# SonyCSLParis/interactive-spectrogram-inpainting

Hardware: AMD Instinct MI355X
Metric: spectrograms/sec VQ-VAE fwd+quantize @B64 (higher is better)
Workload: dtype f32 (products split into two f16 pieces, three terms); 1 GPU; VQVAE.forward (encode + quantize x2 + decode), eval, default ctor (128 hidden, 2 res blocks, D=64, K=512, factors 4/2); batch_per_gpu=64, input=[2,128,512] fp32 randn, weights=random init, codebooks calibrated on encoder outputs, parallelism=replicas x1 (no data-path collective)

## Files before the change

interactive-spectrogram-inpainting_amd/csrc/convT_pair_f16.hip:

```cpp
#include "isi_common.h"
#include "isi_internal.h"
#include "knobs.h"
#include "prof.h"
#include "split_f16.h"

namespace isi {

namespace {

typedef float f32x16 __attribute__((ext_vector_type(16)));
typedef int i32x4 __attribute__((ext_vector_type(4)));
typedef short s16x8 __attribute__((ext_vector_type(8)));
typedef unsigned u32x2v __attribute__((ext_vector_type(2)));
using f16s::f16x8;

constexpr int TW = 64, HWD = TW + 2;
constexpr int ROWB = 64;
constexpr int NPAIR = 8;
constexpr unsigned OOB = 0x7FFFFFF0u, OOB_ST = 0xFFFFFFF0u;

struct ConvTPairK {
  const float *in, *w16, *bias;
  float *out;
  unsigned in_bytes, w_bytes, out_bytes;
  int Cin, Cout, Kpad, H, W, B, relu;
  int tiles_x, tiles_y, ntn;
  const float *w2;
  int n2;
  float *out2;
};

__device__ __forceinline__ void dma16(const unsigned lds_addr, const unsigned voff, const i32x4 rsrc, const unsigned soff) {
  asm volatile("s_mov_b32 m0, %0\n\ts_nop 0\n\tbuffer_load_dwordx4 %1, %2, %3 offen lds"
               :: "s"(lds_addr), "v"(voff), "s"(rsrc), "s"(soff) : "memory");
}
__device__ __forceinline__ i32x4 make_rsrc(const void *ptr, const unsigned bytes) {
  const unsigned long long b = (unsigned long long)ptr;
  return i32x4{(int)(unsigned)b, (int)((unsigned)(b >> 32) & 0xffffu), (int)bytes, 0x00020000};
}
#ifdef ISI_MEASURE
__device__ long long g_convT_pair_stamps[128];
#define ISI_STAMP(i_) do { if (blockIdx.x == 8 && (wave & 3) == 0 && lane == 0 && item_i == (int)blockIdx.x + (int)gridDim.x) \
    g_convT_pair_stamps[(wave >> 2) * 64 + (i_)] = __builtin_readcyclecounter(); } while (0)
#else
#define ISI_STAMP(i_) do { } while (0)
#endif
#define ISI_MH(a_, b_, c_) __builtin_amdgcn_mfma_f32_32x32x16_f16(__builtin_bit_cast(f16x8, a_), __builtin_bit_cast(f16x8, b_), c_, 0, 0, 0)

template <int TH, bool OUTP, bool YP = false>
__global__ __launch_bounds__(TH * 64) void convT_pair_kernel(const ConvTPairK p) {
  constexpr int NW = TH;
  constexpr int HPIX = (TH + 1) * HWD;
  constexpr int A_ROWS = (HPIX + 15) / 16 * 16;
  constexpr int NA = A_ROWS / 16, NWD = NPAIR * 64 / 16;
  constexpr int A_BYTES = A_ROWS * ROWB, W_BYTES = NPAIR * 64 * ROWB, STAGE = A_BYTES + W_BYTES + 1024;
  constexpr int NS = 2;
  constexpr int NDMA = NA + NWD;
  constexpr int PER = (NDMA + NW - 1) / NW;
  extern __shared__ __attribute__((aligned(16))) char smem[];

  const int tid = threadIdx.x, lane = tid & 63;
  const int wave = __builtin_amdgcn_readfirstlane(tid >> 6);
  const int frow = lane & 31, kb = lane >> 5;
  const int Cin = p.Cin, nstage = Cin / 16;
  const i32x4 rsi = make_rsrc(p.in, p.in_bytes), rsw = make_rsrc(p.w16, p.w_bytes);
  const __amdgpu_buffer_rsrc_t rso_b = __builtin_amdgcn_make_buffer_rsrc(p.out, 0, p.out_bytes, 0x00020000);
  const __amdgpu_buffer_rsrc_t rso2_b = __builtin_amdgcn_make_buffer_rsrc(p.out2, 0, p.out2 ? p.out_bytes : 0u, 0x00020000);
  const unsigned lds0 = (unsigned)(size_t)(__attribute__((address_space(3))) char *)smem;
  const int OW = 2 * p.W, OH = 2 * p.H;

  float *bias_s = reinterpret_cast<float *>(smem + NS * STAGE);
  for (int i = tid; i < p.Cout; i += NW * 64) bias_s[i] = p.bias ? p.bias[i] : 0.f;
  unsigned short *w2s = reinterpret_cast<unsigned short *>(bias_s + 64);
  if constexpr (YP) {
    for (int i = tid; i < 4 * 2 * 64 * 8; i += NW * 64) {
      const int e = i & 7, l = (i >> 3) & 63, plane = (i >> 9) & 1, s_ = i >> 10;
      const int n = l & 31, kbl = l >> 5;
      const int ch = 32 * (s_ >> 1) + 16 * (s_ & 1) + (e < 4 ? 4 * kbl + e : 8 + 4 * kbl + (e - 4));
      const float w = n < p.n2 ? p.w2[n * 64 + ch] * f16s::kScaleB : 0.f;
      const _Float16 hi = (_Float16)w;
      const _Float16 v = plane ? (_Float16)(w - (float)hi) : hi;
      w2s[i] = __builtin_bit_cast(unsigned short, v);
    }
  }

  const int per_b = p.tiles_x * p.tiles_y * 2 * p.ntn;
  const int nitems = per_b * p.B;
  for (int item_i = blockIdx.x; item_i < nitems; item_i += gridDim.x) {
    int item;
    {
      const int q = nitems / 8, r = nitems % 8, xcd = item_i % 8, idx = item_i / 8;
      item = (xcd < r ? xcd * (q + 1) : r * (q + 1) + (xcd - r) * q) + idx;
    }
    const int b = item / per_b;
    int rem = item - b * per_b;
    const int tile = rem / (2 * p.ntn);
    rem -= tile * (2 * p.ntn);
    const int py = rem / p.ntn, n0 = (rem - py * p.ntn) * 64;
    const int y0 = (tile / p.tiles_x) * TH, x0 = (tile % p.tiles_x) * TW;
    ISI_STAMP(0);
    __syncthreads();
    ISI_STAMP(1);

    unsigned dvo[PER];
#pragma unroll
    for (int q = 0; q < PER; ++q) {
      const int d = wave + NW * q;
      const int row = (d < NA ? d : d - NA) * 16 + (lane >> 2);
      if (d < NA) {
        const int hy = row / HWD, hx = row - hy * HWD;
        const unsigned piece = (unsigned)(((lane & 3) ^ ((hx >> 2) & 3)) * 16);
        const int gy = y0 - 1 + py + hy, gx = x0 - 1 + hx;
        const bool ok = row < HPIX && (unsigned)gy < (unsigned)p.H && (unsigned)gx < (unsigned)p.W;
        dvo[q] = ok ? (unsigned)(((b * p.H + gy) * p.W + gx) * Cin) * 4u + piece : OOB;
      } else if (d < NDMA) {
        const unsigned piece = (unsigned)(((lane & 3) ^ ((row >> 2) & 3)) * 16);
        const int sl = row >> 6, n = row & 63;
        const int px = sl >> 2, tap = sl & 3;
        dvo[q] = (unsigned)((((py * 2 + px) * p.Cout + n0 + n) * p.Kpad) + tap * Cin) * 4u + piece;
      } else {
        dvo[q] = OOB;
      }
    }
    auto issue = [&](const int stage, const int c16, const int q) {
      const int d = wave + NW * q;
      const bool is_w = d >= NA;
      const unsigned dst = d < NDMA ? (unsigned)(d * 1024) : (unsigned)(A_BYTES + W_BYTES);
      dma16(lds0 + (unsigned)(stage * STAGE) + dst, dvo[q], is_w && d < NDMA ? rsw : rsi, d < NDMA ? (unsigned)(c16 * 64) : 0u);
    };

    const int ry = wave;
    unsigned abase[3][2];
#pragma unroll
    for (int sx = 0; sx < 3; ++sx) {
// ... 93 lines not shown
      for (int px = 0; px < 2; ++px)
#pragma unroll
        for (int i = 0; i < 2; ++i) {
          f32x16 y;
#pragma unroll
          for (int r = 0; r < 16; ++r) y[r] = 0.f;
#pragma unroll
          for (int s_ = 0; s_ < 4; ++s_) {
            const int j = s_ >> 1, qa = 2 * (s_ & 1);
            float u4[8];
#pragma unroll
            for (int e = 0; e < 8; ++e) {
              const int q = qa + (e >> 2);
              const float bv = bias_s[32 * j + 8 * q + 4 * kb + (e & 3)];
              float t = __builtin_fmaf(acc[px][i][j][4 * q + (e & 3)], f16s::kUnscale * f16s::kScaleA, bv * f16s::kScaleA);
              if (p.relu) t = t < 0.f ? 0.f : t;
              u4[e] = t;
            }
            uint4 uh, ul;
            f16s::split2_scaled(u4[0], u4[1], uh.x, ul.x);
            f16s::split2_scaled(u4[2], u4[3], uh.y, ul.y);
            f16s::split2_scaled(u4[4], u4[5], uh.z, ul.z);
            f16s::split2_scaled(u4[6], u4[7], uh.w, ul.w);
            const s16x8 uhv = __builtin_bit_cast(s16x8, uh), ulv = __builtin_bit_cast(s16x8, ul);
            y = ISI_MH(wfh[s_], ulv, y);
            y = ISI_MH(wfl[s_], uhv, y);
            y = ISI_MH(wfh[s_], uhv, y);
          }
          const int gx = x0 + 32 * i + frow;
          const bool ok = gy < p.H && gx < p.W;
          const unsigned o = (unsigned)(((b * OH + 2 * gy + py) * OW + 2 * gx + px) * 32);
#pragma unroll
          for (int q = 0; q < 4; ++q) {
            const uint4 w = make_uint4(__builtin_bit_cast(unsigned, y[4 * q] * f16s::kUnscale), __builtin_bit_cast(unsigned, y[4 * q + 1] * f16s::kUnscale),
                                       __builtin_bit_cast(unsigned, y[4 * q + 2] * f16s::kUnscale), __builtin_bit_cast(unsigned, y[4 * q + 3] * f16s::kUnscale));
            const unsigned off = ok ? (o + (unsigned)(8 * q + 4 * kb)) * 4u : OOB_ST;
            __builtin_amdgcn_raw_buffer_store_b128(__builtin_bit_cast(i32x4, w), rso_b, off, 0, 0);
          }
        }
    } else {
#pragma unroll
    for (int px = 0; px < 2; ++px)
#pragma unroll
      for (int i = 0; i < 2; ++i) {
        const int gx = x0 + 32 * i + frow;
        const bool ok = gy < p.H && gx < p.W;
        const unsigned o = (unsigned)(((b * OH + 2 * gy + py) * OW + 2 * gx + px) * p.Cout + n0);
#pragma unroll
        for (int j = 0; j < 2; ++j)
#pragma unroll
          for (int q = 0; q < 4; ++q) {
            const int cg = 32 * j + 8 * q;
            const float4 bq = *reinterpret_cast<const float4 *>(bias_s + n0 + cg + 4 * kb);
            float v[4];
#pragma unroll
            for (int e = 0; e < 4; ++e) {
              float t = __builtin_fmaf(acc[px][i][j][4 * q + e], f16s::kUnscale, e == 0 ? bq.x : e == 1 ? bq.y : e == 2 ? bq.z : bq.w);
              if (p.relu) t = t < 0.f ? 0.f : t;
              v[e] = t;
            }
            uint4 w;
            unsigned off;
            if constexpr (OUTP) {
              uint2 hi, lo;
              f16s::split4(make_float4(v[0], v[1], v[2], v[3]), f16s::kScaleA, hi, lo);
              const u32x2v sx_ = __builtin_amdgcn_permlane32_swap(hi.x, lo.x, false, false);
              const u32x2v sy_ = __builtin_amdgcn_permlane32_swap(hi.y, lo.y, false, false);
              w = make_uint4(sx_.x, sy_.x, sx_.y, sy_.y);
              off = ok ? (o + (unsigned)cg) * 4u + (unsigned)kb * 16u : OOB_ST;
              if (p.out2) {
                const uint4 wf = make_uint4(__builtin_bit_cast(unsigned, v[0]), __builtin_bit_cast(unsigned, v[1]),
                                            __builtin_bit_cast(unsigned, v[2]), __builtin_bit_cast(unsigned, v[3]));
                __builtin_amdgcn_raw_buffer_store_b128(__builtin_bit_cast(i32x4, wf), rso2_b,
                                                       ok ? (o + (unsigned)(cg + 4 * kb)) * 4u : OOB_ST, 0, 0);
              }
            } else {
              w = make_uint4(__builtin_bit_cast(unsigned, v[0]), __builtin_bit_cast(unsigned, v[1]),
                             __builtin_bit_cast(unsigned, v[2]), __builtin_bit_cast(unsigned, v[3]));
              off = ok ? (o + (unsigned)(cg + 4 * kb)) * 4u : OOB_ST;
            }
            __builtin_amdgcn_raw_buffer_store_b128(__builtin_bit_cast(i32x4, w), rso_b, off, 0, 0);
          }
      }
    }
    ISI_STAMP(5);
  }
}
#undef ISI_MH

template <int TH, bool OUTP, bool YP = false>
int launch_convT_pair(const ConvTPairK &a, hipStream_t stream) {
  constexpr int HPIX = (TH + 1) * HWD;
  constexpr int A_ROWS = (HPIX + 15) / 16 * 16;
  constexpr int NS = 2;
  constexpr size_t ring = (size_t)NS * (A_ROWS * ROWB + NPAIR * 64 * ROWB + 1024);
  static_assert(ring + 4096 <= 160 * 1024, "LDS budget");
  const size_t smem = ring + (size_t)(a.Cout > 64 ? a.Cout : 64) * sizeof(float) + (YP ? 8192 : 0);
  auto kern = convT_pair_kernel<TH, OUTP, YP>;
  static DeviceOnce attr_set;
  if (!attr_set.done()) {
    if (hipFuncSetAttribute(reinterpret_cast<const void *>(kern), hipFuncAttributeMaxDynamicSharedMemorySize, (int)smem) != hipSuccess)
      return check_launch("hipFuncSetAttribute(convT_pair)");
    attr_set.mark();
  }
  const int n_cu = current_device_cu_count();
  const int nitems = a.tiles_x * a.tiles_y * 2 * a.ntn * a.B;
  const double M = (double)a.B * a.H * a.W;
  const double flops = 2.0 * M * 4 * a.Cout * 4.0 * a.Cin;
  const double bytes = 4.0 * (M * a.Cin + 4.0 * M * a.Cout + 16.0 * a.Cin * a.Cout);
  prof::Scope scope(prof::K_CONV_F16X3, flops, bytes, stream);
  ISI_PROF_LAUNCH(scope, kern, dim3(nitems < n_cu ? nitems : n_cu), dim3(TH * 64), smem, stream, a);
  return check_launch("convT_pair_f16");
}

}

bool decoder_tail_ok(int Cin, int Cmid, int Cout) {
  return !knobs().no_tail_fusion && convT_pair_ok(Cin, Cmid) && Cmid == 64 && Cout >= 1 && Cout <= 2;
}

int decoder_tail_f32(const float *in_pair, const float *packed_w1, const float *bias1, const float *packed_w2,
                     const float *bias2, float *yprime_ws, const isi_dst *dst, int B, int H, int W, int Cin, int Cmid,
                     int Cout, hipStream_t stream) {
  if (!in_pair || !packed_w1 || !packed_w2 || !yprime_ws || !dst || !dst->ptr) return invalid("decoder_tail: null pointer");
  if (B <= 0 || H <= 0 || W <= 0) return invalid("decoder_tail: bad shape");
  if (!convT_pair_ok(Cin, Cmid) || Cmid != 64 || Cout < 1 || Cout > 2) return unsupported("decoder_tail: Cin % 16 == 0, Cmid == 64, Cout <= 2");
  const size_t Kpad = round_up((size_t)4 * Cin, kBK);
  int rc = convT_pair_f16(in_pair, packed_w1 + (size_t)4 * Cmid * Kpad, bias1, yprime_ws, B, H, W, Cin, Cmid,  1,
                           0, stream, packed_w2, 16 * Cout);
// ... 3 lines not shown
}

int convT_pair_debug_stamps(long long *host, int n) {
#ifdef ISI_MEASURE
  return hipMemcpyFromSymbol(host, HIP_SYMBOL(g_convT_pair_stamps), sizeof(long long) * (size_t)(n < 128 ? n : 128)) == hipSuccess ? 0 : -2;
#else
  (void)host; (void)n;
  return unsupported("phase timestamps need a -DISI_MEASURE build");
#endif
}

bool convT_pair_ok(int Cin, int Cout) {
  return !knobs().no_convt_pair_kernel && Cin >= 16 && Cin % 16 == 0 && Cout % 64 == 0 && Cout <= 1024;
}

int convT_pair_f16(const float *in, const float *w16, const float *bias, float *out, int B, int H, int W, int Cin,
                   int Cout, int relu, int out_pair, hipStream_t stream, const float *w2, int n2, float *twin) {
  if (!convT_pair_ok(Cin, Cout)) return unsupported("convT_pair: shape outside the fused kernel");
  if (twin && (!out_pair || w2)) return unsupported("convT_pair: an fp32 twin accompanies a pair-format output");
  if (w2 && (Cout != 64 || n2 < 1 || n2 > 32 || out_pair)) return unsupported("convT_pair: the tail form needs Cout == 64 and n2 <= 32");
  const int64_t ein = (int64_t)B * H * W * Cin, eout = (int64_t)B * 4 * H * W * (w2 ? 32 : Cout);
  if (ein * 4 >= 0x70000000ll || eout * 4 >= 0xF0000000ll) return unsupported("convT_pair: tensor too large for 32-bit offsets");
  ConvTPairK a;
  memset(&a, 0, sizeof a);
  a.in = in; a.w16 = w16; a.bias = bias; a.out = out;
  a.Cin = Cin; a.Cout = Cout; a.Kpad = (int)round_up((size_t)4 * Cin, kBK);
  a.in_bytes = (unsigned)(ein * 4); a.out_bytes = (unsigned)(eout * 4);
  a.w_bytes = (unsigned)((size_t)4 * Cout * a.Kpad * 4);
  a.H = H; a.W = W; a.B = B; a.relu = relu;
  a.tiles_x = (W + TW - 1) / TW;
  a.ntn = Cout / 64;
  a.w2 = w2; a.n2 = n2; a.out2 = twin;
  const int forced = knobs().convt_pair_th;
  const long items8 = (long)a.tiles_x * ((H + 7) / 8) * 2 * a.ntn * B;
  const bool th8 = forced == 8 || (forced != 4 && items8 >= 256);
  if (th8) {
    a.tiles_y = (H + 7) / 8;
    if (w2) return launch_convT_pair<8, false, true>(a, stream);
    return out_pair ? launch_convT_pair<8, true>(a, stream) : launch_convT_pair<8, false>(a, stream);
  }
  a.tiles_y = (H + 3) / 4;
  if (w2) return launch_convT_pair<4, false, true>(a, stream);
  return out_pair ? launch_convT_pair<4, true>(a, stream) : launch_convT_pair<4, false>(a, stream);
}

}
```

interactive-spectrogram-inpainting_amd/csrc/conv_igemm_f32.hip:

```cpp
#include <cstdlib>

#include "isi_common.h"
#include "isi_internal.h"
#include "knobs.h"
#include "prof.h"
#include "split_f16.h"

namespace isi {

typedef float f32x16 __attribute__((ext_vector_type(16)));

typedef int i32x4 __attribute__((ext_vector_type(4)));

struct ConvKArgs {
  const float *in0, *in1, *w, *bias, *res;
  float *out;
  unsigned in0_bytes, in1_bytes, w_bytes, out_bytes, res_bytes;
  int C0, Cin, src_uniform;
  int s0n, s0c, s0h, s0w;
  int s1n, s1h, s1w;
  int rn, rc, rh, rw;
  int on, oc, oh, ow;
  int H, W, OH, OW, Cout, K, Kpad, KW, stride, relu, M;
  int bf16x3;
// ... 712 lines not shown
  a.H = H; a.W = W; a.OH = H; a.OW = W; a.Cout = Cout;
  a.K = 4 * a.Cin; a.Kpad = (int)round_up(a.K, kBK);
  a.w_phase_stride = Cout * a.Kpad;
  a.w_bytes = (unsigned)((size_t)4 * Cout * a.Kpad * 4);
  a.KW = 2; a.stride = 1; a.relu = relu & 1; a.bf16x3 = split_mode(relu); a.M = B * H * W;
  a.KH = 2;
  a.in0_pair = (relu & ISI_CONV_IN0_PAIR) ? 1 : 0; a.out_pair = (relu & ISI_CONV_OUT_PAIR) ? 1 : 0;
  a.w16 = (relu & ISI_CONV_W16) ? packed_w + (size_t)4 * Cout * a.Kpad : nullptr;
  a.convT = 1;
  const bool vec = s->sc == 1 && (a.C0 % 4 == 0) && aligned16(s->ptr) && (s->sn % 4 == 0) &&
                   (s->sh % 4 == 0) && (s->sw % 4 == 0);
  if (!aligned16(packed_w)) return invalid("convT: packed weight must be 16-byte aligned");
  return launch_conv(a, !vec, 4, stream);
}

}
```

interactive-spectrogram-inpainting_amd/csrc/isi_api.cpp:

```cpp
#include "isi_common.h"
#include <atomic>
#include <cstdlib>
#include <cstring>

#include "isi_internal.h"
#include "knobs.h"
#include "rel_attention.h"
#include "prof.h"

namespace isi {
static std::atomic<const uint64_t *> g_dropout_seed_base{nullptr};
const uint64_t *dropout_seed_base() { return g_dropout_seed_base.load(); }
static thread_local char g_last_error[512] = "";
void set_last_error(const char *msg) {
  strncpy(g_last_error, msg ? msg : "", sizeof g_last_error - 1);
  g_last_error[sizeof g_last_error - 1] = 0;
}

namespace {
struct KnobEntry { const char *name; int Knobs::*field; int dflt; bool measure_only; };
const KnobEntry kKnobTable[] = {
    {"ISI_CONV_FLUSH", &Knobs::conv_flush, 3, false},
    {"ISI_NO_PAIRS", &Knobs::no_pairs, 0, false},
    {"ISI_NO_CONV_FIRST", &Knobs::no_conv_first, 0, false},
    {"ISI_NO_VQ_FUSION", &Knobs::no_vq_fusion, 0, false},
    {"ISI_NO_CONV_PAIR_KERNEL", &Knobs::no_conv_pair_kernel, 0, false},
    {"ISI_NO_RESBLOCK_PAIR_KERNEL", &Knobs::no_resblock_pair_kernel, 0, false},
    {"ISI_NO_CONVT_PAIR_KERNEL", &Knobs::no_convt_pair_kernel, 0, false},
    {"ISI_NO_TAIL_FUSION", &Knobs::no_tail_fusion, 0, false},
    {"ISI_NO_WGRAD_HALO", &Knobs::no_wgrad_halo, 0, false},
    {"ISI_NO_GEMM_KERNEL", &Knobs::no_gemm_kernel, 0, false},
    {"ISI_GEMM_NO_WIDE", &Knobs::gemm_no_wide, 0, false},
    {"ISI_GEMM_NARROW_BELOW", &Knobs::gemm_narrow_below, 0, false},
    {"ISI_CONV_PAIR_BM", &Knobs::conv_pair_bm, 0, false},
    {"ISI_CONV_PAIR_ALL", &Knobs::conv_pair_all, 0, false},
    {"ISI_RESPAIR_TH", &Knobs::respair_th, 0, false},
    {"ISI_RES_TH", &Knobs::res_th, 0, false},
    {"ISI_CONVT_TH", &Knobs::convt_th, 0, false},
    {"ISI_CONVT_PAIR_TH", &Knobs::convt_pair_th, 0, false},
    {"ISI_DECODE_NT", &Knobs::decode_nt, 1, false},
// ... 493 lines not shown
```

interactive-spectrogram-inpainting_amd/csrc/isi_internal.h:

```cpp
#pragma once
#include <hip/hip_runtime.h>

#include "isi_hip.h"

namespace isi {

int split_conv_weight_f16(const float *packed, float *out, int64_t n_floats, hipStream_t stream);
int pad_channels4_f32(const float *x, float *out, int B, int C, int H, int W, int64_t sn, int64_t sc, int64_t sh, int64_t sw,
                      hipStream_t st);
int add_gate_rows_f32(float *out, const float *a, int64_t lda, const float *b, const float *y, int64_t M, int C, hipStream_t st);
int vq_bwd_rows_f32(float *dz, const float *dq, int64_t ldq, const float *z, const float *q_st, const float *g_diff, int64_t M,
                    int D, hipStream_t st);
int pack_multi(const void *table_dev, int n, int blocks_per_entry, hipStream_t stream);
bool conv_wgrad_halo_route(int Cout, int C0, int C1, int KH, int KW, int stride, int pad, int OH, int OW);
int reduce_jobs_f32(const isi_reduce_job *jobs, int n_jobs, hipStream_t stream);
int64_t adam_num_chunks(const isi_adam_tensor *tensors, int n_tensors);
int grad_sumsq_f32(const isi_adam_tensor *tensors, int n_tensors, float *partials, int64_t n_partials, hipStream_t stream);
int grad_clip_coef_f32(const float *partials, int64_t n_partials, float max_norm, float *norm_coef, hipStream_t stream);
int adam_step_f32(const isi_adam_tensor *tensors, int n_tensors, const isi_adam_hyper *hyper, int n_groups, const float *coef,
                  hipStream_t stream);
int conv_wgrad_deferred_f32(const isi_src *s0, const isi_src *s1, const float *dy, float *dw, int cin_keep, float *db,
                            float *workspace, size_t workspace_floats, int B, int H, int W, int Cout, int KH, int KW, int stride,
                            int pad, int flags, hipStream_t stream, isi_reduce_job *jobs_out, int *n_jobs);
int pair_encode_f32(const float *x, float *out, int64_t n, hipStream_t stream);
// ... 16 lines not shown
  int out_pair;
  float *twin;
};
bool conv_pair_kernel_ok(int C0, int C1, int Cout, int taps);
int conv_pair_f16(const PairConvArgs &c, hipStream_t stream);
int conv_pair_debug_stamps(long long *host, int n);
bool convT_pair_ok(int Cin, int Cout);
bool decoder_tail_ok(int Cin, int Cmid, int Cout);
int decoder_tail_f32(const float *in_pair, const float *packed_w1, const float *bias1, const float *packed_w2,
                     const float *bias2, float *yprime_ws, const isi_dst *dst, int B, int H, int W, int Cin, int Cmid,
                     int Cout, hipStream_t stream);
int convT_pair_debug_stamps(long long *host, int n);
int convT_pair_f16(const float *in, const float *w16, const float *bias, float *out, int B, int H, int W, int Cin,
                   int Cout, int relu, int out_pair, hipStream_t stream, const float *w2 = nullptr, int n2 = 0,
                   float *twin = nullptr);
int conv2d_f32(const isi_src *s0, const isi_src *s1, const float *packed_w, const float *bias,
               const isi_src *res, const isi_dst *dst, int B, int H, int W, int Cout, int KH,
               int KW, int stride, int pad, int relu, hipStream_t stream, const float *gate = nullptr,
               float *twin = nullptr);
int conv2d_batched_f32(const isi_src *s0, const isi_src *s1, const float *packed_w, const float *bias,
                       const isi_src *res, const isi_dst *dst, int B, int H, int W, int Cout, int KH,
                       int KW, int stride, int pad, int relu, int nz, int64_t zs_in0, int64_t zs_w,
                       int64_t zs_res, int64_t zs_out, hipStream_t stream, const float *gate = nullptr,
                       float *twin = nullptr);
int conv_transpose2d_k4s2_f32(const isi_src *s, const float *packed_w, const float *bias,
                              const isi_dst *dst, int B, int H, int W, int Cout, int relu,
                              hipStream_t stream, const float *gate = nullptr, float *twin = nullptr);

bool resblock_fusable(int C, int R);
bool resblock_pair_ok(int C, int R);
bool resblock_pair_preferred(int B, int H, int W, int C, int R);
int resblock_pair_debug_stamps(long long *host, int n);
int resblock_pair_f16(const float *in, const float *w1_16, const float *b1, const float *w2_16, const float *b2, float *out,
                      int B, int H, int W, int C, int relu, int out_pair, hipStream_t stream, float *twin = nullptr,
                      float *hidden = nullptr);
int resblock_f32(const float *in, const float *w1, const float *b1, const float *w2, const float *b2,
                 float *out, int B, int H, int W, int C, int R, int relu, hipStream_t stream, float *twin = nullptr,
                 float *hidden = nullptr);
bool convT_small_applicable(int Cin, int Cout);
bool convT_small_pair_ok(int Cin, int Cout);
int convT_gather_f32(const float *yprime, const float *bias, float *out, int B, int H, int W, int Cout, int on, int oc,
                     int oh, int ow, int relu, hipStream_t stream);
// ... 221 lines not shown
```

interactive-spectrogram-inpainting_amd/csrc/knobs.h:

```cpp
#pragma once

namespace isi {

struct Knobs {
  int conv_flush;
  int no_pairs;
  int no_conv_first;
  int no_vq_fusion;
  int no_conv_pair_kernel;
  int no_resblock_pair_kernel;
  int no_convt_pair_kernel;
  int no_tail_fusion;
  int no_gemm_kernel;
  int gemm_narrow_below;
  int gemm_no_wide;
  int no_wgrad_halo;
  int conv_pair_bm;
  int conv_pair_all;
  int respair_th, res_th, convt_th, convt_pair_th;
  int decode_nt;
  int attn_g_from_kv;
  int wgrad_split_target;
  int attn_full_zero;
  int attn_no_fwd3;
// ... 14 lines not shown
```

interactive-spectrogram-inpainting_amd/csrc/vqvae_run.cpp:

```cpp
#include <algorithm>

#include <cstdlib>
#include "isi_common.h"
#include "isi_internal.h"
#include "knobs.h"

namespace isi {

namespace {

struct Act {
  float *p;
  int C, H, W;
  size_t elems(int B) const { return (size_t)B * H * W * C; }
};

isi_src src_nhwc(const float *p, int C, int H, int W, int Wstride = -1) {
  if (Wstride < 0) Wstride = W;
  isi_src s;
  s.ptr = p; s.C = C; s.sc = 1; s.sw = C; s.sh = (int64_t)Wstride * C; s.sn = (int64_t)H * Wstride * C;
  return s;
}
isi_dst dst_nhwc(float *p, int C, int H, int W) {
  isi_dst d;
// ... 125 lines not shown
  {
    float *o = (e.n_res == 0) ? final_out : ((cur.p == s0) ? s1 : s0);
    isi_dst d = dst_nhwc(o, e.conv3.Cout, cur.H, cur.W);
    stack_pairs = res_stack_in_pairs(pairs, e.n_res, e.res3, B, cur.H, cur.W, e.conv3.Cout);
    int rc = conv2d_f32(&cs, nullptr, e.conv3.w, e.conv3.bias, nullptr, &d, B, cur.H, cur.W,
                        e.conv3.Cout, 3, 3, 1, 1, 1 | pf | (cp ? ISI_CONV_IN0_PAIR : 0) | ((e.n_res && !stack_pairs) ? 0 : op), st);
    if (rc) return rc;
    cur = Act{o, e.conv3.Cout, cur.H, cur.W};
  }
  int rc = run_res_stack(e.n_res, e.res3, e.res1, cur, B, s0, s1, hid, final_out, pf, stack_pairs, pairs, st);
  if (rc) return rc;
  out = cur;
  return ISI_OK;
}

int run_decoder(const isi_decoder_w &d, const isi_src &in0, const isi_src *in1, int B, int H, int W,
                float *s0, float *s1, float *hid, const isi_dst &final_dst, int pf, bool in0_pair, bool in1_pair,
                bool pairs, bool final_pair, hipStream_t st) {
  Act cur{s0, d.conv3.Cout, H, W};
  bool stack_pairs = false;
  auto up_reads_pair = [&](int i, int Cin) {
    if (!pairs) return false;
    if (!convT_small_applicable(Cin, d.up[i].Cout)) return true;
    const bool last = (i == d.n_up - 1);
    return convT_small_pair_ok(Cin, d.up[i].Cout) && last && !final_pair && (pf & ISI_CONV_F16X3) && (pf & ISI_CONV_W16);
  };
  {
    isi_dst dd = dst_nhwc(cur.p, cur.C, H, W);
    stack_pairs = res_stack_in_pairs(pairs, d.n_res, d.res3, B, H, W, cur.C);
    const bool op = d.n_res ? stack_pairs : (d.n_up ? up_reads_pair(0, cur.C) : final_pair);
    int rc = conv2d_f32(&in0, in1, d.conv3.w, d.conv3.bias, nullptr, &dd, B, H, W, cur.C, 3, 3, 1,
                        1, 1 | pf | (in0_pair ? ISI_CONV_IN0_PAIR : 0) | (in1_pair ? ISI_CONV_IN1_PAIR : 0) |
                        (op ? ISI_CONV_OUT_PAIR : 0), st);
// ... 6 lines not shown
    if (rc) return rc;
  }
  for (int i = 0; i < d.n_up; ++i) {
    const bool last = (i == d.n_up - 1);
    isi_src s = src_nhwc(cur.p, cur.C, cur.H, cur.W);
    float *o = (cur.p == s0) ? s1 : s0;
    if (i == d.n_up - 2 && cp && !final_pair && (pf & ISI_CONV_F16X3) && (pf & ISI_CONV_W16) &&
        decoder_tail_ok(cur.C, d.up[i].Cout, d.up[i + 1].Cout)) {
      int rc = decoder_tail_f32(cur.p, d.up[i].w, d.up[i].bias, d.up[i + 1].w, d.up[i + 1].bias, o, &final_dst, B, cur.H,
                                cur.W, cur.C, d.up[i].Cout, d.up[i + 1].Cout, st);
      if (rc) return rc;
      return ISI_OK;
    }
    isi_dst dd = last ? final_dst : dst_nhwc(o, d.up[i].Cout, 2 * cur.H, 2 * cur.W);
    const bool op = last ? final_pair : up_reads_pair(i + 1, d.up[i].Cout);
    int rc = conv_transpose2d_k4s2_f32(&s, d.up[i].w, d.up[i].bias, &dd, B, cur.H, cur.W,
                                       d.up[i].Cout, (last ? 0 : 1) | pf | (cp ? ISI_CONV_IN0_PAIR : 0) |
                                       (op ? ISI_CONV_OUT_PAIR : 0), st);
    if (rc) return rc;
    cp = op;
    cur = Act{o, d.up[i].Cout, 2 * cur.H, 2 * cur.W};
  }
  return ISI_OK;
}

bool stack_fusable(int C, int n_res, const isi_conv_w *res3) {
  for (int i = 0; i < n_res; ++i)
    if (!resblock_fusable(C, res3[i].Cout)) return false;
  return true;
}
bool encoder_pairs_ok(const isi_encoder_w &e, int Cin, bool in_pair) {
  int C = Cin;
  bool cp = in_pair;
// ... 103 lines not shown
  int64_t *id_t = out->id_t ? out->id_t : id_t_ws;
  int64_t *id_b = out->id_b ? out->id_b : id_b_ws;
  float *scal = out->scalars ? out->scalars : scal_ws;
  int rc;
  const int f16 = ISI_CONV_F16X3 | (w.w16 ? ISI_CONV_W16 : 0);
  const int pf_enc = w.precision == 4 ? f16 : w.precision == 3 ? ISI_CONV_BF16X6
                   : w.precision == 2 ? ISI_CONV_BF16X3 : 0;
  const bool pairs = pairs_eligible(w);
  const int pf_dec = w.precision == 4 ? f16 : w.precision >= 1 ? ISI_CONV_BF16X3 : 0;
  const bool fuse_vq = pairs && !w.no_quantize && !knobs().no_vq_fusion;
  const bool frag_packed = fuse_vq && w.w16 == 2 && (mode & ISI_MODE_ENCODE);
  if (frag_packed) {
    rc = vq_zero_counts(counts, 2 * Kmax, st);
    if (rc) return rc;
  }
  bool bottom_pair_done = false;
  bool top_deferred = false;
  int64_t N_top = 0;

  if (mode & ISI_MODE_ENCODE) {
    if (!x) return invalid("vqvae: x is null");
    Act eb, et;
    rc = run_encoder(w.enc_b, src_nchw(x, w.in_channel, H, W), B, H, W, s0, s1, hid, enc_b, eb, pf_enc, false, pairs, st);
    if (rc) return rc;
    rc = run_encoder(w.enc_t, src_nhwc(eb.p, eb.C, eb.H, eb.W), B, eb.H, eb.W, s0, s1, hid, enc_t, et, pf_enc, pairs,
                     pairs, st);
    if (rc) return rc;
    {
      isi_src s = src_nhwc(et.p, et.C, et.H, et.W);
      if (fuse_vq && vq_conv1x1_fusable(et.C, 0, D, w.quantize_t.K)) {
// ... 12 lines not shown
      rc = w.no_quantize ? unquantized_scalars(scal + 0, st)
                         : run_quantizer(w.quantize_t, zbuf, (int64_t)B * et.H * et.W, id_t, quant_t, counts_top,
                                         sse_part, scal + 0, pf_enc & ISI_CONV_F16X3, st);
      if (rc) return rc;
      if (pairs) {
        rc = pair_encode_f32(quant_t, q_t_pair, (int64_t)B * et.H * et.W * D, st);
        if (rc) return rc;
      }
    }
  top_done:;
    int Wd = et.W;
    for (int i = 0; i < w.dec_t.n_up; ++i) Wd *= 2;
    {
      isi_src s = src_nhwc(pairs ? q_t_pair : quant_t, D, et.H, et.W);
      isi_dst d = dst_nhwc(dec_t, w.dec_t.up[w.dec_t.n_up - 1].Cout, sh.Hb, Wd);
      rc = run_decoder(w.dec_t, s, nullptr, B, et.H, et.W, s0, s1, hid, d, pf_enc, pairs, false, pairs, pairs, st);
      if (rc) return rc;
    }
    {
      const int Cd = w.dec_t.up[w.dec_t.n_up - 1].Cout;
      isi_src a = src_nhwc(dec_t, Cd, sh.Hb, sh.Wq, Wd);
      isi_src b = src_nhwc(eb.p, eb.C, sh.Hb, sh.Wq, eb.W);
      if (fuse_vq && vq_conv1x1_fusable(Cd, eb.C, D, w.quantize_b.K)) {
        rc = run_quantizer_fused(w.quantize_b, w.quantize_conv_b, a, &b, B, sh.Hb, sh.Wq, id_b,
                                 (out->quant_b || !(mode & ISI_MODE_DECODE)) ? quant_b : nullptr, q_b_pair, counts,
                                 sse_part, scal + 2, wfrag_ws, st,  !top_deferred, frag_packed);
        if (rc) return rc;
        if (top_deferred) {
          const int64_t N_b = (int64_t)B * sh.Hb * sh.Wq;
          rc = vq_finalize2_f32(sse_top, vq_num_partials(N_top), counts_top, w.quantize_t.K, N_top, sse_part,
                                vq_num_partials(N_b), counts, w.quantize_b.K, N_b, D, scal, st);
// ... 31 lines not shown
    }
    if (!bottom_pair_done) {
      rc = pair_encode_f32(quant_b, q_b_pair, (int64_t)B * sh.Hb * sh.Wq * D, st);
      if (rc) return rc;
    }
  }

  if (mode & ISI_MODE_DECODE) {
    if (!out->dec) return invalid("vqvae: dec output is null");
    if (!(mode & ISI_MODE_ENCODE) && (!out->quant_t || !out->quant_b))
      return invalid("vqvae: decode needs quant_t and quant_b");
    const float *cur = pairs ? q_t_pair : quant_t;
    int h = sh.Ht, ww = sh.Wt;
    for (int i = 0; i < w.n_upsample; ++i) {
      float *o = (i % 2 == 0) ? up : up2;
      isi_src s = src_nhwc(cur, w.upsample[i].Cin, h, ww);
      isi_dst d = dst_nhwc(o, w.upsample[i].Cout, 2 * h, 2 * ww);
      rc = conv_transpose2d_k4s2_f32(&s, w.upsample[i].w, w.upsample[i].bias, &d, B, h, ww,
                                     w.upsample[i].Cout, pf_dec | (pairs ? ISI_CONV_IN0_PAIR | ISI_CONV_OUT_PAIR : 0), st);
      if (rc) return rc;
      cur = o; h *= 2; ww *= 2;
    }
    if (h != sh.Hb || ww != sh.Wq) return invalid("vqvae: upsampled top grid != bottom grid");
    isi_src a = src_nhwc(cur, D, h, ww);
    isi_src b = src_nhwc(pairs ? q_b_pair : quant_b, D, sh.Hb, sh.Wq);
    int OHf = sh.Hb, OWf = sh.Wq;
    for (int i = 0; i < w.dec.n_up; ++i) { OHf *= 2; OWf *= 2; }
    isi_dst d = dst_nchw(out->dec, w.in_channel, OHf, OWf);
    rc = run_decoder(w.dec, a, &b, B, sh.Hb, sh.Wq, s0, s1, hid, d, pf_dec, pairs, pairs, pairs, false, st);
    if (rc) return rc;
// ... 28 lines not shown
```

Before: 37350 spectrograms/s.

## Group top-decoder and upsample transposed convs into one paired kernel launch

Adds a grouped variant of the pair-format transposed-conv kernel that processes two independent problems in one launch, interleaving work items from each across a persistent grid. In forward mode, the top decoder's upsampling convT is launched together with the matching upsample-path convT, which reads the same quantized top codes. Those upsample layers are then skipped in the decode stage. The aim is to fill the GPU better and cut launch count for small layers. The cost is per-item selection of parameters, which may raise register pressure, plus extra routing logic with a fallback when shapes differ.

```diff
diff --git a/interactive-spectrogram-inpainting_amd/csrc/convT_pair_f16.hip b/interactive-spectrogram-inpainting_amd/csrc/convT_pair_f16.hip
--- a/interactive-spectrogram-inpainting_amd/csrc/convT_pair_f16.hip
+++ b/interactive-spectrogram-inpainting_amd/csrc/convT_pair_f16.hip
@@ -29,6 +29,15 @@
   int n2;
   float *out2;
 };
+struct ConvTPairK2 {
+  ConvTPairK a, b;
+};
+template <int NP> struct ConvTPairArg { typedef ConvTPairK type; };
+template <> struct ConvTPairArg<2> { typedef ConvTPairK2 type; };
+__device__ __forceinline__ const ConvTPairK &problem0(const ConvTPairK &p) { return p; }
+__device__ __forceinline__ const ConvTPairK &problem1(const ConvTPairK &p) { return p; }
+__device__ __forceinline__ const ConvTPairK &problem0(const ConvTPairK2 &g) { return g.a; }
+__device__ __forceinline__ const ConvTPairK &problem1(const ConvTPairK2 &g) { return g.b; }
 
 __device__ __forceinline__ void dma16(const unsigned lds_addr, const unsigned voff, const i32x4 rsrc, const unsigned soff) {
   asm volatile("s_mov_b32 m0, %0\n\ts_nop 0\n\tbuffer_load_dwordx4 %1, %2, %3 offen lds"
@@ -47,8 +56,12 @@
 #endif
 #define ISI_MH(a_, b_, c_) __builtin_amdgcn_mfma_f32_32x32x16_f16(__builtin_bit_cast(f16x8, a_), __builtin_bit_cast(f16x8, b_), c_, 0, 0, 0)
 
-template <int TH, bool OUTP, bool YP = false>
-__global__ __launch_bounds__(TH * 64) void convT_pair_kernel(const ConvTPairK p) {
+template <int TH, bool OUTP, bool YP = false, int NP = 1>
+__global__ __launch_bounds__(TH * 64) void convT_pair_kernel(const typename ConvTPairArg<NP>::type g) {
+  static_assert(NP == 1 || (NP == 2 && OUTP && !YP), "grouped launches: plain pair-format layers only");
+  const ConvTPairK &p = problem0(g);
+  const ConvTPairK &p1 = problem1(g);
+#define ISI_F(f_) (NP == 2 && sel ? p1.f_ : p.f_)
   constexpr int NW = TH;
   constexpr int HPIX = (TH + 1) * HWD;
   constexpr int A_ROWS = (HPIX + 15) / 16 * 16;
@@ -62,15 +75,13 @@
   const int tid = threadIdx.x, lane = tid & 63;
   const int wave = __builtin_amdgcn_readfirstlane(tid >> 6);
   const int frow = lane & 31, kb = lane >> 5;
-  const int Cin = p.Cin, nstage = Cin / 16;
-  const i32x4 rsi = make_rsrc(p.in, p.in_bytes), rsw = make_rsrc(p.w16, p.w_bytes);
-  const __amdgpu_buffer_rsrc_t rso_b = __builtin_amdgcn_make_buffer_rsrc(p.out, 0, p.out_bytes, 0x00020000);
-  const __amdgpu_buffer_rsrc_t rso2_b = __builtin_amdgcn_make_buffer_rsrc(p.out2, 0, p.out2 ? p.out_bytes : 0u, 0x00020000);
   const unsigned lds0 = (unsigned)(size_t)(__attribute__((address_space(3))) char *)smem;
   const int OW = 2 * p.W, OH = 2 * p.H;
 
   float *bias_s = reinterpret_cast<float *>(smem + NS * STAGE);
   for (int i = tid; i < p.Cout; i += NW * 64) bias_s[i] = p.bias ? p.bias[i] : 0.f;
+  if constexpr (NP == 2)
+    for (int i = tid; i < p1.Cout; i += NW * 64) bias_s[p.Cout + i] = p1.bias ? p1.bias[i] : 0.f;
   unsigned short *w2s = reinterpret_cast<unsigned short *>(bias_s + 64);
   if constexpr (YP) {
     for (int i = tid; i < 4 * 2 * 64 * 8; i += NW * 64) {
@@ -84,9 +95,31 @@
     }
   }
 
-  const int per_b = p.tiles_x * p.tiles_y * 2 * p.ntn;
-  const int nitems = per_b * p.B;
-  for (int item_i = blockIdx.x; item_i < nitems; item_i += gridDim.x) {
+  const int G = (int)gridDim.x;
+  const int n_p0 = p.tiles_x * p.tiles_y * 2 * p.ntn * p.B;
+  int cnt0 = 0, cnt1 = 0, w1 = 0;
+  if constexpr (NP == 2) {
+    const int n_p1 = p.tiles_x * p.tiles_y * 2 * p1.ntn * p.B;
+    w1 = ((int)blockIdx.x - n_p0 % G + G) % G;
+    cnt0 = n_p0 > (int)blockIdx.x ? (n_p0 - (int)blockIdx.x - 1) / G + 1 : 0;
+    cnt1 = n_p1 > w1 ? (n_p1 - w1 - 1) / G + 1 : 0;
+  }
+  const int cmin = cnt0 < cnt1 ? cnt0 : cnt1;
+  for (int k = 0, item_i = (int)blockIdx.x; NP == 2 ? k < cnt0 + cnt1 : item_i < n_p0; ++k, item_i += G) {
+    int sel = 0;
+    if constexpr (NP == 2) {
+      const int kk = k < 2 * cmin ? k >> 1 : k - cmin;
+      sel = k < 2 * cmin ? k & 1 : (cnt1 > cnt0 ? 1 : 0);
+      item_i = (sel ? w1 : (int)blockIdx.x) + kk * G;
+    }
+    const int Cin = ISI_F(Cin), nstage = Cin / 16, Cout = ISI_F(Cout), ntn = ISI_F(ntn), Kpad = ISI_F(Kpad);
+    const int relu = ISI_F(relu);
+    const i32x4 rsi = make_rsrc(ISI_F(in), ISI_F(in_bytes)), rsw = make_rsrc(ISI_F(w16), ISI_F(w_bytes));
+    const __amdgpu_buffer_rsrc_t rso_b = __builtin_amdgcn_make_buffer_rsrc(ISI_F(out), 0, ISI_F(out_bytes), 0x00020000);
+    const __amdgpu_buffer_rsrc_t rso2_b = __builtin_amdgcn_make_buffer_rsrc(p.out2, 0, p.out2 ? p.out_bytes : 0u, 0x00020000);
+    const float *bias_i = NP == 2 && sel ? bias_s + p.Cout : bias_s;
+    const int per_b = p.tiles_x * p.tiles_y * 2 * ntn;
+    const int nitems = per_b * p.B;
     int item;
     {
       const int q = nitems / 8, r = nitems % 8, xcd = item_i % 8, idx = item_i / 8;
@@ -94,9 +127,9 @@
     }
     const int b = item / per_b;
     int rem = item - b * per_b;
-    const int tile = rem / (2 * p.ntn);
-    rem -= tile * (2 * p.ntn);
-    const int py = rem / p.ntn, n0 = (rem - py * p.ntn) * 64;
+    const int tile = rem / (2 * ntn);
+    rem -= tile * (2 * ntn);
+    const int py = rem / ntn, n0 = (rem - py * ntn) * 64;
     const int y0 = (tile / p.tiles_x) * TH, x0 = (tile % p.tiles_x) * TW;
     ISI_STAMP(0);
     __syncthreads();
@@ -117,7 +150,7 @@
         const unsigned piece = (unsigned)(((lane & 3) ^ ((row >> 2) & 3)) * 16);
         const int sl = row >> 6, n = row & 63;
         const int px = sl >> 2, tap = sl & 3;
-        dvo[q] = (unsigned)((((py * 2 + px) * p.Cout + n0 + n) * p.Kpad) + tap * Cin) * 4u + piece;
+        dvo[q] = (unsigned)((((py * 2 + px) * Cout + n0 + n) * Kpad) + tap * Cin) * 4u + piece;
       } else {
         dvo[q] = OOB;
       }
@@ -241,7 +274,7 @@
               const int q = qa + (e >> 2);
               const float bv = bias_s[32 * j + 8 * q + 4 * kb + (e & 3)];
               float t = __builtin_fmaf(acc[px][i][j][4 * q + (e & 3)], f16s::kUnscale * f16s::kScaleA, bv * f16s::kScaleA);
-              if (p.relu) t = t < 0.f ? 0.f : t;
+              if (relu) t = t < 0.f ? 0.f : t;
               u4[e] = t;
             }
             uint4 uh, ul;
@@ -272,18 +305,18 @@
       for (int i = 0; i < 2; ++i) {
         const int gx = x0 + 32 * i + frow;
         const bool ok = gy < p.H && gx < p.W;
-        const unsigned o = (unsigned)(((b * OH + 2 * gy + py) * OW + 2 * gx + px) * p.Cout + n0);
+        const unsigned o = (unsigned)(((b * OH + 2 * gy + py) * OW + 2 * gx + px) * Cout + n0);
 #pragma unroll
         for (int j = 0; j < 2; ++j)
 #pragma unroll
           for (int q = 0; q < 4; ++q) {
             const int cg = 32 * j + 8 * q;
-            const float4 bq = *reinterpret_cast<const float4 *>(bias_s + n0 + cg + 4 * kb);
+            const float4 bq = *reinterpret_cast<const float4 *>(bias_i + n0 + cg + 4 * kb);
             float v[4];
 #pragma unroll
             for (int e = 0; e < 4; ++e) {
               float t = __builtin_fmaf(acc[px][i][j][4 * q + e], f16s::kUnscale, e == 0 ? bq.x : e == 1 ? bq.y : e == 2 ? bq.z : bq.w);
-              if (p.relu) t = t < 0.f ? 0.f : t;
+              if (relu) t = t < 0.f ? 0.f : t;
               v[e] = t;
             }
             uint4 w;
@@ -295,7 +328,7 @@
               const u32x2v sy_ = __builtin_amdgcn_permlane32_swap(hi.y, lo.y, false, false);
               w = make_uint4(sx_.x, sy_.x, sx_.y, sy_.y);
               off = ok ? (o + (unsigned)cg) * 4u + (unsigned)kb * 16u : OOB_ST;
-              if (p.out2) {
+              if (NP == 1 && p.out2) {
                 const uint4 wf = make_uint4(__builtin_bit_cast(unsigned, v[0]), __builtin_bit_cast(unsigned, v[1]),
                                             __builtin_bit_cast(unsigned, v[2]), __builtin_bit_cast(unsigned, v[3]));
                 __builtin_amdgcn_raw_buffer_store_b128(__builtin_bit_cast(i32x4, wf), rso2_b,
@@ -314,6 +347,7 @@
   }
 }
 #undef ISI_MH
+#undef ISI_F
 
 template <int TH, bool OUTP, bool YP = false>
 int launch_convT_pair(const ConvTPairK &a, hipStream_t stream) {
@@ -340,6 +374,35 @@
   return check_launch("convT_pair_f16");
 }
 
+template <int TH>
+int launch_convT_pair2(const ConvTPairK2 &g, hipStream_t stream) {
+  constexpr int HPIX = (TH + 1) * HWD;
+  constexpr int A_ROWS = (HPIX + 15) / 16 * 16;
+  constexpr int NS = 2;
+  constexpr size_t ring = (size_t)NS * (A_ROWS * ROWB + NPAIR * 64 * ROWB + 1024);
+  static_assert(ring + 4096 <= 160 * 1024, "LDS budget");
+  const int nbias = g.a.Cout + g.b.Cout;
+  const size_t smem = ring + (size_t)(nbias > 64 ? nbias : 64) * sizeof(float);
+  auto kern = convT_pair_kernel<TH, true, false, 2>;
+  static DeviceOnce attr_set;
+  if (!attr_set.done()) {
+    if (hipFuncSetAttribute(reinterpret_cast<const void *>(kern), hipFuncAttributeMaxDynamicSharedMemorySize, (int)(ring + 4096)) != hipSuccess)
+      return check_launch("hipFuncSetAttribute(convT_pair, grouped)");
+    attr_set.mark();
+  }
+  const int n_cu = current_device_cu_count();
+  const long nitems = (long)g.a.tiles_x * g.a.tiles_y * 2 * (g.a.ntn + g.b.ntn) * g.a.B;
+  const double M = (double)g.a.B * g.a.H * g.a.W;
+  double flops = 0, bytes = 0;
+  for (const ConvTPairK *a : {&g.a, &g.b}) {
+    flops += 2.0 * M * 4 * a->Cout * 4.0 * a->Cin;
+    bytes += 4.0 * (M * a->Cin + 4.0 * M * a->Cout + 16.0 * a->Cin * a->Cout);
+  }
+  prof::Scope scope(prof::K_CONV_F16X3, flops, bytes, stream);
+  ISI_PROF_LAUNCH(scope, kern, dim3((unsigned)(nitems < n_cu ? nitems : n_cu)), dim3(TH * 64), smem, stream, g);
+  return check_launch("convT_pair_f16 (grouped)");
+}
+
 }
 
 bool decoder_tail_ok(int Cin, int Cmid, int Cout) {
@@ -373,14 +436,10 @@
   return !knobs().no_convt_pair_kernel && Cin >= 16 && Cin % 16 == 0 && Cout % 64 == 0 && Cout <= 1024;
 }
 
-int convT_pair_f16(const float *in, const float *w16, const float *bias, float *out, int B, int H, int W, int Cin,
-                   int Cout, int relu, int out_pair, hipStream_t stream, const float *w2, int n2, float *twin) {
-  if (!convT_pair_ok(Cin, Cout)) return unsupported("convT_pair: shape outside the fused kernel");
-  if (twin && (!out_pair || w2)) return unsupported("convT_pair: an fp32 twin accompanies a pair-format output");
-  if (w2 && (Cout != 64 || n2 < 1 || n2 > 32 || out_pair)) return unsupported("convT_pair: the tail form needs Cout == 64 and n2 <= 32");
+static int convT_pair_describe(ConvTPairK &a, bool *th8, const float *in, const float *w16, const float *bias, float *out, int B,
+                               int H, int W, int Cin, int Cout, int relu, const float *w2, int n2, float *twin) {
   const int64_t ein = (int64_t)B * H * W * Cin, eout = (int64_t)B * 4 * H * W * (w2 ? 32 : Cout);
   if (ein * 4 >= 0x70000000ll || eout * 4 >= 0xF0000000ll) return unsupported("convT_pair: tensor too large for 32-bit offsets");
-  ConvTPairK a;
   memset(&a, 0, sizeof a);
   a.in = in; a.w16 = w16; a.bias = bias; a.out = out;
   a.Cin = Cin; a.Cout = Cout; a.Kpad = (int)round_up((size_t)4 * Cin, kBK);
@@ -392,15 +451,42 @@
   a.w2 = w2; a.n2 = n2; a.out2 = twin;
   const int forced = knobs().convt_pair_th;
   const long items8 = (long)a.tiles_x * ((H + 7) / 8) * 2 * a.ntn * B;
-  const bool th8 = forced == 8 || (forced != 4 && items8 >= 256);
+  *th8 = forced == 8 || (forced != 4 && items8 >= 256);
+  a.tiles_y = *th8 ? (H + 7) / 8 : (H + 3) / 4;
+  return ISI_OK;
+}
+
+int convT_pair_f16(const float *in, const float *w16, const float *bias, float *out, int B, int H, int W, int Cin,
+                   int Cout, int relu, int out_pair, hipStream_t stream, const float *w2, int n2, float *twin) {
+  if (!convT_pair_ok(Cin, Cout)) return unsupported("convT_pair: shape outside the fused kernel");
+  if (twin && (!out_pair || w2)) return unsupported("convT_pair: an fp32 twin accompanies a pair-format output");
+  if (w2 && (Cout != 64 || n2 < 1 || n2 > 32 || out_pair)) return unsupported("convT_pair: the tail form needs Cout == 64 and n2 <= 32");
+  ConvTPairK a;
+  bool th8;
+  if (int rc = convT_pair_describe(a, &th8, in, w16, bias, out, B, H, W, Cin, Cout, relu, w2, n2, twin)) return rc;
   if (th8) {
-    a.tiles_y = (H + 7) / 8;
     if (w2) return launch_convT_pair<8, false, true>(a, stream);
     return out_pair ? launch_convT_pair<8, true>(a, stream) : launch_convT_pair<8, false>(a, stream);
   }
-  a.tiles_y = (H + 3) / 4;
   if (w2) return launch_convT_pair<4, false, true>(a, stream);
   return out_pair ? launch_convT_pair<4, true>(a, stream) : launch_convT_pair<4, false>(a, stream);
 }
 
-}
+int convT_pair2_f16(const float *const in[2], const float *const w16[2], const float *const bias[2], float *const out[2],
+                    int B, int H, int W, const int Cin[2], const int Cout[2], const int relu[2], hipStream_t stream) {
+  if (!convT_pair_ok(Cin[0], Cout[0]) || !convT_pair_ok(Cin[1], Cout[1]) || Cout[0] + Cout[1] > 1024)
+    return unsupported("convT_pair2: shape outside the fused kernel");
+  ConvTPairK2 g;
+  bool th8[2];
+  const int first = Cin[1] > Cin[0] ? 1 : 0;
+  for (int i = 0; i < 2; ++i) {
+    const int j = i ^ first;
+    if (int rc = convT_pair_describe(i ? g.b : g.a, &th8[i], in[j], w16[j], bias[j], out[j], B, H, W, Cin[j], Cout[j], relu[j],
+                                     nullptr, 0, nullptr))
+      return rc;
+  }
+  if (th8[0] != th8[1]) return unsupported("convT_pair2: the two problems take different tile heights");
+  return th8[0] ? launch_convT_pair2<8>(g, stream) : launch_convT_pair2<4>(g, stream);
+}
+
+}
diff --git a/interactive-spectrogram-inpainting_amd/csrc/conv_igemm_f32.hip b/interactive-spectrogram-inpainting_amd/csrc/conv_igemm_f32.hip
--- a/interactive-spectrogram-inpainting_amd/csrc/conv_igemm_f32.hip
+++ b/interactive-spectrogram-inpainting_amd/csrc/conv_igemm_f32.hip
@@ -750,4 +750,37 @@
   return launch_conv(a, !vec, 4, stream);
 }
 
-}
+static bool convT_routes_to_pair_kernel(const ConvTProblem &p, int B, int H, int W) {
+  if (!p.s || !p.s->ptr || !p.packed_w || !p.dst || !p.dst->ptr || p.Cout <= 0) return false;
+  const isi_src *s = p.s;
+  const isi_dst *dst = p.dst;
+  const int Cin = s->C, Cout = p.Cout;
+  if ((int64_t)B * H * W > INT32_MAX) return false;
+  if (extent(B, s->sn, Cin, s->sc, H, s->sh, W, s->sw) > kMaxElems ||
+      extent(B, dst->sn, Cout, dst->sc, 2 * H, dst->sh, 2 * W, dst->sw) > kMaxElems) return false;
+  if (convT_small_applicable(Cin, Cout)) return false;
+  const bool dense_in = s->sc == 1 && (W == 1 || s->sw == Cin) && (H == 1 || s->sh == (int64_t)W * Cin) &&
+                        (B == 1 || s->sn == (int64_t)H * W * Cin);
+  const bool dense_out = dst->sc == 1 && dst->sw == Cout && dst->sh == (int64_t)2 * W * Cout &&
+                         (B == 1 || dst->sn == (int64_t)4 * H * W * Cout);
+  return (p.flags & ISI_CONV_IN0_PAIR) && (p.flags & ISI_CONV_OUT_PAIR) && (p.flags & ISI_CONV_W16) && split_mode(p.flags) == 3 &&
+         dense_in && dense_out && convT_pair_ok(Cin, Cout) && aligned16(s->ptr) && aligned16(dst->ptr) && aligned16(p.packed_w);
+}
+
+int conv_transpose2d_k4s2_pair2_f32(const ConvTProblem &p0, const ConvTProblem &p1, int B, int H, int W, hipStream_t stream) {
+  if (B <= 0 || H <= 0 || W <= 0) return invalid("convT: bad shape");
+  if (!convT_routes_to_pair_kernel(p0, B, H, W) || !convT_routes_to_pair_kernel(p1, B, H, W))
+    return unsupported("convT: the grouped launch takes two layers of the fused pair kernel, pairs in and out");
+  const ConvTProblem *p[2] = {&p0, &p1};
+  const float *in[2], *w16[2], *bias[2];
+  float *out[2];
+  int Cin[2], Cout[2], relu[2];
+  for (int i = 0; i < 2; ++i) {
+    in[i] = p[i]->s->ptr; Cin[i] = p[i]->s->C; Cout[i] = p[i]->Cout; relu[i] = p[i]->flags & 1;
+    w16[i] = p[i]->packed_w + (size_t)4 * Cout[i] * round_up((size_t)4 * Cin[i], kBK);
+    bias[i] = p[i]->bias; out[i] = p[i]->dst->ptr;
+  }
+  return convT_pair2_f16(in, w16, bias, out, B, H, W, Cin, Cout, relu, stream);
+}
+
+}
diff --git a/interactive-spectrogram-inpainting_amd/csrc/isi_api.cpp b/interactive-spectrogram-inpainting_amd/csrc/isi_api.cpp
--- a/interactive-spectrogram-inpainting_amd/csrc/isi_api.cpp
+++ b/interactive-spectrogram-inpainting_amd/csrc/isi_api.cpp
@@ -24,6 +24,7 @@
     {"ISI_NO_PAIRS", &Knobs::no_pairs, 0, false},
     {"ISI_NO_CONV_FIRST", &Knobs::no_conv_first, 0, false},
     {"ISI_NO_VQ_FUSION", &Knobs::no_vq_fusion, 0, false},
+    {"ISI_NO_CONVT_GROUP", &Knobs::no_convt_group, 0, false},
     {"ISI_NO_CONV_PAIR_KERNEL", &Knobs::no_conv_pair_kernel, 0, false},
     {"ISI_NO_RESBLOCK_PAIR_KERNEL", &Knobs::no_resblock_pair_kernel, 0, false},
     {"ISI_NO_CONVT_PAIR_KERNEL", &Knobs::no_convt_pair_kernel, 0, false},
diff --git a/interactive-spectrogram-inpainting_amd/csrc/isi_internal.h b/interactive-spectrogram-inpainting_amd/csrc/isi_internal.h
--- a/interactive-spectrogram-inpainting_amd/csrc/isi_internal.h
+++ b/interactive-spectrogram-inpainting_amd/csrc/isi_internal.h
@@ -54,6 +54,8 @@
 int convT_pair_f16(const float *in, const float *w16, const float *bias, float *out, int B, int H, int W, int Cin,
                    int Cout, int relu, int out_pair, hipStream_t stream, const float *w2 = nullptr, int n2 = 0,
                    float *twin = nullptr);
+int convT_pair2_f16(const float *const in[2], const float *const w16[2], const float *const bias[2], float *const out[2],
+                    int B, int H, int W, const int Cin[2], const int Cout[2], const int relu[2], hipStream_t stream);
 int conv2d_f32(const isi_src *s0, const isi_src *s1, const float *packed_w, const float *bias,
                const isi_src *res, const isi_dst *dst, int B, int H, int W, int Cout, int KH,
                int KW, int stride, int pad, int relu, hipStream_t stream, const float *gate = nullptr,
@@ -66,6 +68,13 @@
 int conv_transpose2d_k4s2_f32(const isi_src *s, const float *packed_w, const float *bias,
                               const isi_dst *dst, int B, int H, int W, int Cout, int relu,
                               hipStream_t stream, const float *gate = nullptr, float *twin = nullptr);
+struct ConvTProblem {
+  const isi_src *s;
+  const float *packed_w, *bias;
+  const isi_dst *dst;
+  int Cout, flags;
+};
+int conv_transpose2d_k4s2_pair2_f32(const ConvTProblem &p0, const ConvTProblem &p1, int B, int H, int W, hipStream_t stream);
 
 bool resblock_fusable(int C, int R);
 bool resblock_pair_ok(int C, int R);
diff --git a/interactive-spectrogram-inpainting_amd/csrc/knobs.h b/interactive-spectrogram-inpainting_amd/csrc/knobs.h
--- a/interactive-spectrogram-inpainting_amd/csrc/knobs.h
+++ b/interactive-spectrogram-inpainting_amd/csrc/knobs.h
@@ -7,6 +7,7 @@
   int no_pairs;
   int no_conv_first;
   int no_vq_fusion;
+  int no_convt_group;
   int no_conv_pair_kernel;
   int no_resblock_pair_kernel;
   int no_convt_pair_kernel;
diff --git a/interactive-spectrogram-inpainting_amd/csrc/vqvae_run.cpp b/interactive-spectrogram-inpainting_amd/csrc/vqvae_run.cpp
--- a/interactive-spectrogram-inpainting_amd/csrc/vqvae_run.cpp
+++ b/interactive-spectrogram-inpainting_amd/csrc/vqvae_run.cpp
@@ -163,9 +163,13 @@
   return ISI_OK;
 }
 
+struct ConvTPartners {
+  ConvTProblem level[ISI_MAX_STAGES];
+  int n, done;
+};
 int run_decoder(const isi_decoder_w &d, const isi_src &in0, const isi_src *in1, int B, int H, int W,
                 float *s0, float *s1, float *hid, const isi_dst &final_dst, int pf, bool in0_pair, bool in1_pair,
-                bool pairs, bool final_pair, hipStream_t st) {
+                bool pairs, bool final_pair, hipStream_t st, ConvTPartners *partners = nullptr) {
   Act cur{s0, d.conv3.Cout, H, W};
   bool stack_pairs = false;
   auto up_reads_pair = [&](int i, int Cin) {
@@ -202,9 +206,16 @@
     }
     isi_dst dd = last ? final_dst : dst_nhwc(o, d.up[i].Cout, 2 * cur.H, 2 * cur.W);
     const bool op = last ? final_pair : up_reads_pair(i + 1, d.up[i].Cout);
-    int rc = conv_transpose2d_k4s2_f32(&s, d.up[i].w, d.up[i].bias, &dd, B, cur.H, cur.W,
-                                       d.up[i].Cout, (last ? 0 : 1) | pf | (cp ? ISI_CONV_IN0_PAIR : 0) |
-                                       (op ? ISI_CONV_OUT_PAIR : 0), st);
+    const int flags = (last ? 0 : 1) | pf | (cp ? ISI_CONV_IN0_PAIR : 0) | (op ? ISI_CONV_OUT_PAIR : 0);
+    int rc = ISI_E_UNSUPPORTED;
+    if (partners && partners->done == i && i < partners->n) {
+      const ConvTProblem mine{&s, d.up[i].w, d.up[i].bias, &dd, d.up[i].Cout, flags};
+      rc = conv_transpose2d_k4s2_pair2_f32(mine, partners->level[i], B, cur.H, cur.W, st);
+      if (rc == ISI_OK) partners->done = i + 1;
+      else if (rc != ISI_E_UNSUPPORTED) return rc;
+    }
+    if (rc == ISI_E_UNSUPPORTED)
+      rc = conv_transpose2d_k4s2_f32(&s, d.up[i].w, d.up[i].bias, &dd, B, cur.H, cur.W, d.up[i].Cout, flags, st);
     if (rc) return rc;
     cp = op;
     cur = Act{o, d.up[i].Cout, 2 * cur.H, 2 * cur.W};
@@ -338,6 +349,11 @@
     rc = vq_zero_counts(counts, 2 * Kmax, st);
     if (rc) return rc;
   }
+  const bool group_up = pairs && mode == ISI_MODE_FORWARD && !knobs().no_convt_group;
+  ConvTPartners up_partners;
+  up_partners.n = up_partners.done = 0;
+  isi_src up_src[ISI_MAX_STAGES];
+  isi_dst up_dst[ISI_MAX_STAGES];
   bool bottom_pair_done = false;
   bool top_deferred = false;
   int64_t N_top = 0;
@@ -380,7 +396,20 @@
     {
       isi_src s = src_nhwc(pairs ? q_t_pair : quant_t, D, et.H, et.W);
       isi_dst d = dst_nhwc(dec_t, w.dec_t.up[w.dec_t.n_up - 1].Cout, sh.Hb, Wd);
-      rc = run_decoder(w.dec_t, s, nullptr, B, et.H, et.W, s0, s1, hid, d, pf_enc, pairs, false, pairs, pairs, st);
+      if (group_up) {
+        const float *cur = q_t_pair;
+        int h = sh.Ht, ww = sh.Wt;
+        for (int i = 0; i < w.n_upsample; ++i) {
+          up_src[i] = src_nhwc(cur, w.upsample[i].Cin, h, ww);
+          up_dst[i] = dst_nhwc((i % 2 == 0) ? up : up2, w.upsample[i].Cout, 2 * h, 2 * ww);
+          up_partners.level[i] = ConvTProblem{&up_src[i], w.upsample[i].w, w.upsample[i].bias, &up_dst[i], w.upsample[i].Cout,
+                                              pf_dec | ISI_CONV_IN0_PAIR | ISI_CONV_OUT_PAIR};
+          cur = up_dst[i].ptr; h *= 2; ww *= 2;
+        }
+        up_partners.n = w.n_upsample;
+      }
+      rc = run_decoder(w.dec_t, s, nullptr, B, et.H, et.W, s0, s1, hid, d, pf_enc, pairs, false, pairs, pairs, st,
+                       group_up ? &up_partners : nullptr);
       if (rc) return rc;
     }
     {
@@ -442,6 +471,10 @@
     int h = sh.Ht, ww = sh.Wt;
     for (int i = 0; i < w.n_upsample; ++i) {
       float *o = (i % 2 == 0) ? up : up2;
+      if (i < up_partners.done) {
+        cur = o; h *= 2; ww *= 2;
+        continue;
+      }
       isi_src s = src_nhwc(cur, w.upsample[i].Cin, h, ww);
       isi_dst d = dst_nhwc(o, w.upsample[i].Cout, 2 * h, 2 * ww);
       rc = conv_transpose2d_k4s2_f32(&s, w.upsample[i].w, w.upsample[i].bias, &d, B, h, ww,
```

Result: no change. 37230 spectrograms/s (-0.3%).
